# KenHBS/LDA_thesis

Hardware: AMD Instinct MI355X
Metric: million tokens resampled/sec (Gibbs sweep) (higher is better)
Workload: dtype f64-exact (fp32 tier 0 + fp64 tiers: the drawn topic is the fp64 pipeline's)

## Files before the change

### lda_thesis_amd/csrc/kernel_quad.hpp

```cpp
#pragma once

namespace {

constexpr float QM_L = 1.05f * 32.0f * 0x1p-24f, QM_T = 1.05f * 39.0f * 0x1p-24f, QM_P = 1.05f * 37.0f * 0x1p-24f, QM_TOT = 1.05f * 0.25f * 0x1p-24f;
#define QLDS(arr, rho, t) (arr)[(rho) >> 2][t][(rho) & 3]
constexpr int QT = 32;
#ifdef LLDA_QUAD_PRIO
constexpr int QP_TOP = (LLDA_QUAD_PRIO) / 100 % 10, QP_DEC = (LLDA_QUAD_PRIO) / 10 % 10, QP_BULK = (LLDA_QUAD_PRIO) % 10;
#else
constexpr int QP_TOP = 3, QP_DEC = 0, QP_BULK = 2;
#endif
constexpr int QNT = 128;
template <bool B> struct QuadForm { static constexpr bool value = B; };

template <int LB>
struct QuadGeo {
    static constexpr int LPD = 1 << LB;
    static constexpr int G = 2 * LPD;
    static constexpr int KP = 32 * LPD;
    static constexpr int IS = 3 + LB;
    static constexpr int DPW = 64 / LPD;
    static constexpr uint64_t GM = LPD == 64 ? ~0ull : ((1ull << LPD) - 1);
};

template <int LB>
__device__ __forceinline__ int quad_rho(int pos) { return ((pos >> LB) & 0x18) | ((pos & 3) << 1) | ((pos >> 2) & 1); }
constexpr int quad_rho_of(int i, int e, int c) { return 8 * i + 2 * c + e; }

constexpr int QK_LANE = 14;
constexpr uint32_t QK_ZN = (1u << QK_LANE) - 1;
template <int LB> constexpr uint32_t QUAD_KEY_NONE = 0x3Fu << QK_LANE | 31u << 9 | (uint32_t)(QuadGeo<LB>::KP - 1);
static_assert((0x3Fu << QK_LANE | QK_ZN) <= 0x7FFFFFFFu, "the key fits 31 bits");

template <int LB>
__device__ __forceinline__ uint32_t quad_min_key(uint32_t key)
{
    if constexpr (LB == 4)
        asm volatile("s_nop 1\n\tv_min_u32_dpp %0, %0, %0 row_ror:8 row_mask:0xf bank_mask:0xf\n\ts_nop 1\n\t"
                     "v_min_u32_dpp %0, %0, %0 row_ror:4 row_mask:0xf bank_mask:0xf\n\ts_nop 1\n\t"
                     "v_min_u32_dpp %0, %0, %0 row_ror:2 row_mask:0xf bank_mask:0xf\n\ts_nop 1\n\t"
                     "v_min_u32_dpp %0, %0, %0 row_ror:1 row_mask:0xf bank_mask:0xf" : "+v"(key));
    else if constexpr (LB == 3)
        asm volatile("s_nop 1\n\tv_min_u32_dpp %0, %0, %0 row_half_mirror row_mask:0xf bank_mask:0xf\n\ts_nop 1\n\t"
                     "v_min_u32_dpp %0, %0, %0 quad_perm:[1,0,3,2] row_mask:0xf bank_mask:0xf\n\ts_nop 1\n\t"
                     "v_min_u32_dpp %0, %0, %0 quad_perm:[2,3,0,1] row_mask:0xf bank_mask:0xf" : "+v"(key));
    else
        asm volatile("s_nop 1\n\tv_min_u32_dpp %0, %0, %0 quad_perm:[1,0,3,2] row_mask:0xf bank_mask:0xf\n\ts_nop 1\n\t"
                     "v_min_u32_dpp %0, %0, %0 quad_perm:[2,3,0,1] row_mask:0xf bank_mask:0xf" : "+v"(key));
    return key;
}

template <int LB>
struct QuadCounts {
    const int (*s_ndk)[QNT][4];
    const int *s_nk0;
    int t;
    int e;
    int g;
    bool st;
    __device__ __forceinline__ int word(int s) const { return QLDS(s_ndk, 8 * (s >> 2) + 2 * (s & 3) + e, t); }
    __device__ __forceinline__ int nd(int s) const { return word(s) & 0xffff; }
    __device__ __forceinline__ int nk(int s) const
    {
        const int w = word(s);
        return s_nk0[pos_of<QuadGeo<LB>::G, 16>(g, s)] + (w & 0xffff) - (int)((uint32_t)w >> 16);
    }
    __device__ __forceinline__ bool stats() const { return st; }
    __device__ __forceinline__ bool count_unsure() const { return false; }
};

template <int LB, bool PAD>
__device__ __noinline__ int quad_cold(const int (*s_ndk)[QNT][4], const int *s_nk0, int tbase, int w, int f, int zo, uint32_t ra,
                                      uint32_t rb, int lane, int64_t d, const KParams *P)
{
    constexpr int G = QuadGeo<LB>::G;
    const int g = lane & (G - 1);
    int x[16];
    gload_lane_row<G, 16>(P->n_kw, (int64_t)w * QuadGeo<LB>::KP, g, x);
    int lo, so;
    lane_slot_of<G, 16>(zo, lo, so);
#pragma unroll
    for (int s = 0; s < 16; ++s) x[s] -= (g == lo && s == so) ? f : 0;
    const QuadCounts<LB> dc{s_ndk, s_nk0, tbase + (g >> 1), g & 1, g, lane < G};
    if constexpr (PAD) return cold_tiers_acc<G, 16, true, false>(dc, x, P->lab_mask[d * G + g], uniform53(ra, rb), g, lane, P);
    else return cold_tiers_acc<G, 16, false, true>(dc, x, 0xFFFFu, uniform53(ra, rb), g, lane, P);
}

typedef float q_v2f __attribute__((ext_vector_type(2)));
typedef float q_v32f __attribute__((ext_vector_type(32)));

template <int LB, bool PAD = false, bool HOOKS = true>
__device__ __forceinline__ uint64_t quad_draw(const q_v32f &xv, const q_v2f (&pa)[16], float u, float margin_rel, float margin_data, float beta,
                                              int lq, int &zn)
{
    const q_v2f b2 = {beta, beta};
    q_v2f Q[16];
    LLDA_MARK("scores");
#pragma unroll
    for (int a = 0; a < 16; ++a) {
        const q_v2f x2 = {xv[2 * a], xv[2 * a + 1]};
        const q_v2f nb = x2 + b2;
        if (a == 0) Q[0] = nb * pa[0];
        else Q[a] = __builtin_elementwise_fma(nb, pa[a], Q[a - 1]);
    }
    LLDA_MARK("lane_scan");
    __builtin_amdgcn_s_setprio(QP_DEC);
    const float X0 = Q[15].x + Q[15].y;
    float X = X0;
    float tot = X0, prev;
    if constexpr (LB == 4) {
        X += dpp_f32<DPP_ROW_SHR + 1>(X);
        X += dpp_f32<DPP_ROW_SHR + 2>(X);
        X += dpp_f32<DPP_ROW_SHR + 4>(X);
        X += dpp_f32<DPP_ROW_SHR + 8>(X);
        tot += dpp_f32<DPP_ROW_ROR + 8>(tot);
        tot += dpp_f32<DPP_ROW_ROR + 4>(tot);
        tot += dpp_f32<DPP_ROW_ROR + 2>(tot);
        tot += dpp_f32<DPP_ROW_ROR + 1>(tot);
        prev = __int_as_float(__builtin_amdgcn_update_dpp(0, __float_as_int(X), DPP_ROW_SHR + 1, 0xF, 0xF, true));
    } else {
        const float m1 = lq >= 1 ? 1.0f : 0.0f, m2 = lq >= 2 ? 1.0f : 0.0f;
        X = __builtin_fmaf(dpp_f32<DPP_ROW_SHR + 1>(X), m1, X);
        X = __builtin_fmaf(dpp_f32<DPP_ROW_SHR + 2>(X), m2, X);
        if constexpr (LB == 3) {
            const float m4 = lq >= 4 ? 1.0f : 0.0f;
            X = __builtin_fmaf(dpp_f32<DPP_ROW_SHR + 4>(X), m4, X);
            tot += dpp_f32<DPP_HALF_MIRROR>(tot);
        }
        tot += dpp_f32<DPP_XOR1>(tot);
        tot += dpp_f32<DPP_XOR2>(tot);
        prev = dpp_f32<DPP_ROW_SHR + 1>(X) * m1;
    }
    LLDA_MARK("threshold");
    const float t = u * tot;
    const float tg = t - prev;
    const float md = __builtin_fmaf(QM_L, X0, __builtin_fmaf(QM_T, t, __builtin_fmaf(QM_P, prev, QM_TOT * tot)));
    float margin = md;
    if constexpr (HOOKS) margin = __builtin_fmaf(tot, margin_rel, margin_data * md);
    const float lo0 = tg - margin, hi0 = tg + margin;
    LLDA_MARK("search");
    const bool c0 = Q[15].x <= lo0;
    const float dA = c0 ? Q[15].x : 0.0f;
    const float lo = lo0 - dA, hi = hi0 - dA;
    float q[16];
#pragma unroll
    for (int a = 0; a < 16; ++a) q[a] = c0 ? Q[a].y : Q[a].x;
    const bool c5 = q[15] <= lo;
    float ub = c5 ? __int_as_float(0x7f800000) : q[15];
    const bool c1 = q[7] <= lo;
    ub = c1 ? ub : q[7];
    const float m2 = c1 ? q[11] : q[3];
    const float a1 = c1 ? q[9] : q[1], a5 = c1 ? q[13] : q[5];
    const float e0 = c1 ? q[8] : q[0], e2 = c1 ? q[10] : q[2], e4 = c1 ? q[12] : q[4], e6 = c1 ? q[14] : q[6];
    const bool c2 = m2 <= lo;
    ub = c2 ? ub : m2;
    const float m3 = c2 ? a5 : a1;
    const float g0 = c2 ? e4 : e0, g2 = c2 ? e6 : e2;
    const bool c3 = m3 <= lo;
    ub = c3 ? ub : m3;
    const float m4 = c3 ? g2 : g0;
    const bool c4 = m4 <= lo;
    ub = c4 ? ub : m4;
    uint64_t bad_total;
    asm("v_cmp_class_f32_e64 %0, %1, %2" : "=s"(bad_total) : "v"(tot - margin), "v"(0x2FF));
    uint64_t unsure = __ballot(!(ub > hi)) | bad_total;
    LLDA_MARK("pick");
    constexpr uint32_t I1 = 2u << QuadGeo<LB>::IS, I0 = 1u << QuadGeo<LB>::IS;
    const uint32_t p = (c1 ? (I1 | 16u << 9) : 0u) | (c2 ? (I0 | 8u << 9) : 0u) | (c3 ? (2u | 4u << 9) : 0u) |
                       (c4 ? (1u | 2u << 9) : 0u) | (c0 ? (4u | 1u << 9) : 0u) | ((uint32_t)lq << 3) | ((uint32_t)lq << QK_LANE);
    uint32_t key = c5 ? QUAD_KEY_NONE<LB> : p;
    key = quad_min_key<LB>(key);
    zn = (int)(key & QK_ZN);
    if constexpr (PAD) unsure |= __ballot(key == QUAD_KEY_NONE<LB>);
    return unsure;
}

template <int LB, bool PAD = false>
__device__ __forceinline__ uint64_t quad_tier1(const q_v32f &xv, const int (*s_ndk)[QNT][4], const int *s_nk0, int tid, int lq, double u,
                                               double alpha, double beta, double vbeta, double margin_rel, uint32_t vm, int &zn)
{
    double W[QT];
    double run = 0.0;
#pragma unroll
    for (int k = 0; k < QT; ++k) {
        const int e = k >> 4, a = k & 15, i = a >> 2, c = a & 3;
        const int rho = quad_rho_of(i, e, c);
        const int w = QLDS(s_ndk, rho, tid);
        const int nd = w & 0xffff, nk = s_nk0[(i << QuadGeo<LB>::IS) | (lq << 3) | (e << 2) | c] + nd - (int)((uint32_t)w >> 16);
        const double den = (double)nk + vbeta;
        double y = (double)__builtin_amdgcn_rcpf((float)den);
        y = __builtin_fma(__builtin_fma(-den, y, 1.0), y, y);
        y = __builtin_fma(__builtin_fma(-den, y, 1.0), y, y);
        const double ws = ((double)nd + alpha) * (((double)xv[rho] + beta) * y);
        run = run + (((vm >> k) & 1u) ? ws : 0.0);
        W[k] = run;
    }
    constexpr int LPD = QuadGeo<LB>::LPD;
    const double X = group_scan<LPD>(run, lq);
    const double tot = bcast_last<LPD>(X, tid & 63);
    double prev = dpp_f64<DPP_ROW_SHR + 1>(X);
    if constexpr (LB < 4) prev = lq ? prev : 0.0;
    const double tg = u * tot - prev;
    const double margin = tot * margin_rel;
    const double lo = tg - margin, hi = tg + margin;
    int cnt_lo = 0, cnt_hi = 0;
#pragma unroll
    for (int k = 0; k < QT; ++k) {
        cnt_lo += (W[k] <= lo) ? 1 : 0;
        cnt_hi += (W[k] <= hi) ? 1 : 0;
    }
    uint64_t unsure = __ballot((cnt_lo != cnt_hi) || !(tot > 0.0) || !(margin < tot));
    const uint32_t k = (uint32_t)cnt_lo;
    const uint32_t i_ = (k >> 2) & 3u, e_ = (k >> 4) & 1u, c_ = k & 3u;
    const uint32_t p = (i_ << QuadGeo<LB>::IS) | ((uint32_t)lq << 3) | (e_ << 2) | c_ | ((8u * i_ + 2u * c_ + e_) << 9) | ((uint32_t)lq << QK_LANE);
    uint32_t key = cnt_lo >= QT ? QUAD_KEY_NONE<LB> : p;
    key = quad_min_key<LB>(key);
    zn = (int)(key & QK_ZN);
    if constexpr (PAD) unsure |= __ballot(key == QUAD_KEY_NONE<LB>);
    return unsure;
}

struct QuadSite { int v, f, zo, c, zn, lo, so; uint8_t w; };

struct QuadDocLds {
    __attribute__((aligned(16))) int ndk[QT / 4][QNT][4];
    __attribute__((aligned(16))) float pa[QT / 4][QNT][4];
};
static_assert(offsetof(QuadDocLds, pa) == sizeof(int) * QT * QNT && sizeof(int) * QT * QNT < 65536,
              "the factor of a slot is an immediate offset away from its count");

#ifdef QUAD_PROFILE
#define QP_DECL uint32_t qp_t = 0, qp_acc[8] = {0, 0, 0, 0, 0, 0, 0, 0}
#define QP_START() do { __builtin_amdgcn_sched_barrier(0); qp_t = (uint32_t)__builtin_amdgcn_s_memtime(); __builtin_amdgcn_sched_barrier(0); } while (0)
#define QP_MARK(k) do { __builtin_amdgcn_sched_barrier(0); const uint32_t qp_n = (uint32_t)__builtin_amdgcn_s_memtime(); \
                        qp_acc[k] += qp_n - qp_t; qp_t = qp_n; __builtin_amdgcn_sched_barrier(0); } while (0)
#else
#define QP_DECL
#define QP_START()
#define QP_MARK(k)
#endif

template <int LB, bool REC = (LB < 4), bool PAD = false, bool HOOKS = false>
__global__ void __launch_bounds__(QNT, 2) llda_sweep_quad_kernel(const KParams P)
{
    typedef QuadGeo<LB> Geo;
    constexpr int KP = Geo::KP, LPD = Geo::LPD, G = Geo::G, IS = Geo::IS;
    __shared__ int s_nk[KP];
    __shared__ int s_nk0[KP];
    __shared__ QuadDocLds s_doc;
    int (*const s_ndk)[QNT][4] = s_doc.ndk;
    float (*const s_pa)[QNT][4] = s_doc.pa;
    __shared__ float s_u[QNT / LPD][2 * LPD];
    __shared__ __attribute__((aligned(16))) int s_hot[QT][16];
    __shared__ uint16_t s_ent[KP];
    static_assert(LB != 4 || sizeof(s_nk) + sizeof(s_nk0) + sizeof(s_doc) + sizeof(s_u) + sizeof(s_hot) + sizeof(s_ent) <= 40960,
                  "K = 512: the static LDS of a workgroup must leave room for four workgroups on a CU");

    const int tid = threadIdx.x;
    for (int i = tid; i < KP; i += QNT) {
        s_nk[i] = 0;
        s_nk0[i] = P.n_k[i];
        s_ent[i] = (uint16_t)quad_rho<LB>(i);
    }
    for (int i = tid; i < QT * 16; i += QNT) {
        const int so = i >> 4, k = i & 15;
        const int kk = ((so & 1) << 3) | ((so >> 4) << 2) | (((so >> 3) & 1) << 1) | ((so >> 2) & 1);
        s_hot[so][k] = k == kk ? -(1 << (((so >> 1) & 1) << 4)) : 0;
    }
    __syncthreads();

    const int lane = tid & 63, lq = tid & (LPD - 1), row = lane >> LB, grp = tid >> LB;
    const int gbase = lane & (64 - LPD);
    const float vbeta32 = (float)P.vbeta, alpha32 = (float)P.alpha, beta32 = (float)P.beta;

    const int64_t site_base = P.doc_off[0];
    const int32_t *word_b = P.word + site_base, *freq_b = P.freq + site_base, *csc_b = P.csc_pos + site_base;
    int32_t *z_b = P.z + site_base;

    typedef int v4i __attribute__((ext_vector_type(4)));
    QP_DECL;

    auto ndk_of = [&](int sg) -> int * { return &QLDS(s_doc.ndk, sg, tid); };
    auto pa_of = [&](int *nd) -> float * { return (float *)((char *)nd + offsetof(QuadDocLds, pa)); };
    auto update = [&](int sg, int pos, int df) {
        int *const c = ndk_of(sg);
        const int w = *c + df;
        *c = w;
        const int nd = w & 0xffff, nk = s_nk0[pos] + nd - (int)((uint32_t)w >> 16);
        *pa_of(c) = tier0_factor(nd, nk, alpha32, vbeta32);
    };

    for (int it = 0; it < P.dpg; ++it) {
        const int64_t idx = ((int64_t)blockIdx.x * P.dpg + it) * (QNT / LPD) + grp;
        const bool valid = idx < P.D;
        const int64_t ic = valid ? idx : P.D - 1;
        const int64_t d = P.doc_order ? (int64_t)P.doc_order[ic] : ic;
        int64_t s0 = P.doc_off[d];
        int len = valid ? (int)(P.doc_off[d + 1] - s0) : 0;
        if (len <= 0) {
            len = 0;
            s0 = site_base;
        }
        int maxlen, minlen;
        if constexpr (LB == 4) {
            const int l0 = __builtin_amdgcn_readlane(len, 0), l1 = __builtin_amdgcn_readlane(len, 16);
            const int l2 = __builtin_amdgcn_readlane(len, 32), l3 = __builtin_amdgcn_readlane(len, 48);
            maxlen = max(max(l0, l1), max(l2, l3));
            minlen = min(min(l0, l1), min(l2, l3));
        } else {
            int ml = len, nl = len;
#pragma unroll
            for (int m = LPD; m < 64; m <<= 1) {
                ml = max(ml, __shfl_xor(ml, m, 64));
                nl = min(nl, __shfl_xor(nl, m, 64));
            }
            maxlen = __builtin_amdgcn_readfirstlane(ml);
            minlen = __builtin_amdgcn_readfirstlane(nl);
        }
        if (maxlen == 0) continue;

        int32_t *ndk_row = P.n_dk + d * KP;
        const uint32_t vm = PAD ? (uint32_t)P.lab_mask[d * G + 2 * lq] | (uint32_t)P.lab_mask[d * G + 2 * lq + 1] << 16 : ~0u;
        {
            int big = 0, tokens = 0;
#pragma unroll
            for (int i = 0; i < 4; ++i) {
                const v4i a = ((const v4i *)ndk_row)[i * G + 2 * lq], b = ((const v4i *)ndk_row)[i * G + 2 * lq + 1];
                const int r[8] = {a.x, a.y, a.z, a.w, b.x, b.y, b.z, b.w};
#pragma unroll
                for (int j = 0; j < 8; ++j) {
                    const int rho = quad_rho_of(i, j >> 2, j & 3);
                    const int k = s_nk0[(i << IS) + lq * 8 + j];
                    QLDS(s_ndk, rho, tid) = r[j] | (r[j] << 16);
                    QLDS(s_pa, rho, tid) = ((vm >> (16 * (j >> 2) + 4 * i + (j & 3))) & 1u) ? tier0_factor(r[j], k, alpha32, vbeta32) : 0.0f;
                    big |= r[j];
                    tokens += (int)((uint32_t)r[j] & 0xffffu);
                }
            }
#pragma unroll
            for (int m = 1; m < LPD; m <<= 1) tokens += __shfl_xor(tokens, m, LPD);
            if (valid && (((uint32_t)big >> 16) || tokens > 65535) && P.status) atomicOr(P.status, 4);
        }
        const uint32_t gdoc = (uint32_t)(d + P.doc_base);
        const uint32_t sb = (uint32_t)(s0 - site_base) * 4u;
        const int last = len > 0 ? len - 1 : 0;
        auto off_of = [&](int n) { return opaque_u32(sb + (uint32_t)min(n, last) * 4u); };
        auto off_full = [&](int n) { return opaque_u32(sb + (uint32_t)n * 4u); };
        auto load_scalars = [&](QuadSite &R, const uint32_t o) {
            R.v = gload_i32(word_b, o); R.f = gload_i32(freq_b, o); R.c = gload_i32(csc_b, o); R.zo = gload_i32(z_b, o);
        };
        const int32_t *rec_b = REC ? P.site_rec + site_base * 4 : nullptr;
        int pv = 0, pf = 0, pc = 0;
        auto load_rec = [&](int &v, int &f, int &c, const uint32_t o) {
            const v4i r = *(const LLDA_GLOBAL v4i *)((const LLDA_GLOBAL char *)rec_b + (o << 2));
            v = r.x; f = r.y; c = r.z;
        };
        auto decode_old = [&](QuadSite &R) {
            R.lo = (R.zo >> 3) & (LPD - 1);
            R.so = s_ent[R.zo];
            asm("" : "+v"(R.so));
        };
        int xp[16];
        auto load_row16 = [&](const int v, uint8_t &flag) {
#ifdef ABL_NOLOAD
#pragma unroll
            for (int k = 0; k < 16; ++k) xp[k] = ((v + k) & 7) * 0x10001;
            flag = 1;
            return;
#endif
            const LLDA_GLOBAL char *q = (const LLDA_GLOBAL char *)P.n_kw16 + (((uint32_t)v << (IS + 3)) + (uint32_t)lq * 16u);
            const v4i a = *(const LLDA_GLOBAL v4i *)q, b = *(const LLDA_GLOBAL v4i *)(q + 32 * LPD);
            const v4i c = *(const LLDA_GLOBAL v4i *)(q + 16 * LPD), e = *(const LLDA_GLOBAL v4i *)(q + 48 * LPD);
            xp[0] = a.x; xp[1] = a.y; xp[2] = a.z; xp[3] = a.w;
            xp[4] = b.x; xp[5] = b.y; xp[6] = b.z; xp[7] = b.w;
            xp[8] = c.x; xp[9] = c.y; xp[10] = c.z; xp[11] = c.w;
            xp[12] = e.x; xp[13] = e.y; xp[14] = e.z; xp[15] = e.w;
            flag = *(const LLDA_GLOBAL uint8_t *)((const LLDA_GLOBAL char *)P.row16 + (uint32_t)v);
        };
        q_v32f xv;
        auto convert_row = [&](const int v, const uint8_t flag, const int so, const float own) {
            LLDA_MARK("convert");
            const uint64_t wide_w = __ballot(flag == 0);
            if (__builtin_expect(wide_w == 0, 1)) {
#pragma unroll
                for (int k = 0; k < 16; ++k) {
                    const int e = k >> 3, j = (k >> 2) & 1, m = k & 3;
                    const int i = 2 * j + (m >> 1), c = 2 * (m & 1);
                    xv[quad_rho_of(i, e, c)] = (float)((uint32_t)xp[k] & 0xffffu);
                    xv[quad_rho_of(i, e, c + 1)] = (float)((uint32_t)xp[k] >> 16);
                }
            } else {
                LLDA_MARK("rare_wide_row");
                int xi[QT];
#pragma unroll
                for (int t = 0; t < QT; ++t) xi[t] = 0;
                if (flag == 0) {
                    const LLDA_GLOBAL v4i *q = (const LLDA_GLOBAL v4i *)((const LLDA_GLOBAL int32_t *)P.n_kw + ((uint64_t)(uint32_t)v << (IS + 2)));
#pragma unroll
                    for (int i = 0; i < 4; ++i) {
                        const v4i a = q[i * G + 2 * lq], b = q[i * G + 2 * lq + 1];
                        xi[quad_rho_of(i, 0, 0)] = a.x; xi[quad_rho_of(i, 0, 1)] = a.y; xi[quad_rho_of(i, 0, 2)] = a.z; xi[quad_rho_of(i, 0, 3)] = a.w;
                        xi[quad_rho_of(i, 1, 0)] = b.x; xi[quad_rho_of(i, 1, 1)] = b.y; xi[quad_rho_of(i, 1, 2)] = b.z; xi[quad_rho_of(i, 1, 3)] = b.w;
                    }
                }
#pragma unroll
                for (int k = 0; k < 16; ++k) {
                    const int e = k >> 3, j = (k >> 2) & 1, m = k & 3;
                    const int i = 2 * j + (m >> 1), c = 2 * (m & 1);
                    const int ra_ = quad_rho_of(i, e, c), rb_ = quad_rho_of(i, e, c + 1);
                    xv[ra_] = flag == 0 ? (float)xi[ra_] : (float)((uint32_t)xp[k] & 0xffffu);
                    xv[rb_] = flag == 0 ? (float)xi[rb_] : (float)((uint32_t)xp[k] >> 16);
                }
#pragma unroll
                for (int r = 0; r < QT; ++r) xv[r] -= (flag == 0 && so == r) ? own : 0.0f;
            }
        };
        auto remove_own_packed = [&](const int so, const int own) {
            LLDA_MARK("own_removal");
            __builtin_assume((uint32_t)own < 65536u);
            const v4i *hot = (const v4i *)&s_hot[so][0];
#pragma unroll
            for (int j = 0; j < 4; ++j) {
                const v4i h = hot[j];
                xp[4 * j] += __mul24(h.x, own); xp[4 * j + 1] += __mul24(h.y, own);
                xp[4 * j + 2] += __mul24(h.z, own); xp[4 * j + 3] += __mul24(h.w, own);
            }
        };

        QuadSite R0, R1, R2;
        int wq = 0;
        if constexpr (REC) {
            load_rec(R0.v, R0.f, R0.c, off_of(0)); R0.zo = gload_i32(z_b, off_of(0));
            load_rec(R1.v, R1.f, R1.c, off_of(1)); R1.zo = gload_i32(z_b, off_of(1));
            load_rec(pv, pf, pc, off_of(2));
        } else {
            load_scalars(R0, off_of(0));
            load_scalars(R1, off_of(1));
            wq = gload_i32(word_b, off_of(2));
        }
        R0.zn = R1.zn = R2.zn = R2.f = R2.c = R2.lo = R2.so = R2.w = 0;
        R2.v = REC ? pv : wq;
        R2.zo = gload_i32(z_b, off_of(2));
        load_row16(R0.v, R0.w);
        uint32_t r0 = 0, r1 = 0, r2 = 0, r3 = 0;
        decode_old(R0);
        decode_old(R1);
        if (len > 0 && lq == R0.lo) update(R0.so, R0.zo, -R0.f);
        remove_own_packed(R0.so, (len > 0 && lq == R0.lo) ? R0.f : 0);
        convert_row(R0.v, R0.w, R0.so, (len > 0 && lq == R0.lo) ? (float)R0.f : 0.0f);
        load_row16(R1.v, R1.w);

        auto site = [&](auto form, const int n, QuadSite &cur, QuadSite &nxt, QuadSite &prv) {
            constexpr bool FULL = decltype(form)::value;
            const bool act = FULL || n < len, more = FULL || n + 1 < len;
            auto off = [&](int m) { if constexpr (FULL) return off_full(m); else return off_of(m); };
            const int f = cur.f, zo = cur.zo;
            QP_START();
            if constexpr (FULL) { LLDA_MARK("site_top"); } else { LLDA_MARK("site_top_masked"); }
            LLDA_MARK("lds_factors");
            __builtin_amdgcn_s_setprio(QP_TOP);
            q_v2f pa[16];
#pragma unroll
            for (int a = 0; a < 16; ++a) {
                pa[a].x = QLDS(s_pa, 2 * a, tid);
                pa[a].y = QLDS(s_pa, 2 * a + 1, tid);
            }
            LLDA_MARK("rng");
            if ((n & (2 * LPD - 1)) == 0) {
                LLDA_MARK("rare_philox");
                r0 = (uint32_t)(n >> 1) + (uint32_t)lq; r1 = gdoc; r2 = P.stream_id; r3 = P.sweep;
                philox4x32_10(r0, r1, r2, r3, P.key0, P.key1);
                s_u[grp][2 * lq] = (float)(r0 >> 5) * 0x1p-27f;
                s_u[grp][2 * lq + 1] = (float)(r2 >> 5) * 0x1p-27f;
                LLDA_MARK("rng");
            }
            const float u32 = s_u[grp][n & (2 * LPD - 1)];
            QP_MARK(0);
            int zn;
            uint64_t unsure;
            if constexpr (HOOKS) unsure = quad_draw<LB, PAD, true>(xv, pa, u32, P.margin0_rel, P.margin0_data, beta32, lq, zn);
            else unsure = quad_draw<LB, PAD, false>(xv, pa, u32, 0.0f, 1.0f, beta32, lq, zn);
            if constexpr (!FULL) unsure &= __ballot(act);
            QP_MARK(1);
            LLDA_MARK("cold_check");
            if (__builtin_expect(unsure != 0, 0)) {
                LLDA_MARK("rare_cold");
                const int holder = (n >> 1) & (LPD - 1);
                const uint32_t ra_l = (n & 1) ? r2 : r0, rb_l = (n & 1) ? r3 : r1;
                const int bp_h = (gbase | holder) << 2;
                const uint32_t ra = (uint32_t)__builtin_amdgcn_ds_bpermute(bp_h, (int)ra_l), rb = (uint32_t)__builtin_amdgcn_ds_bpermute(bp_h, (int)rb_l);
                const uint64_t t0_w = unsure;
                if (lq == 0 && ((t0_w >> gbase) & Geo::GM) && P.status) atomicAdd(P.status + 1, 1);
                int z1;
                uint64_t still = ((!HOOKS || P.margin_rel < 1.0 ? quad_tier1<LB, PAD>(xv, s_ndk, s_nk0, tid, lq, uniform53(ra, rb), P.alpha, P.beta, P.vbeta,
                                                                                  P.margin_rel, vm, z1) : ~0ull) | __ballot(cur.w == 0));
                if constexpr (!FULL) still &= __ballot(act);
                const bool mine0 = ((t0_w >> gbase) & Geo::GM) != 0;
                zn = mine0 ? z1 : zn;
                uint32_t rows = 0;
#pragma unroll
                for (int r = 0; r < Geo::DPW; ++r)
                    rows |= (((t0_w >> (LPD * r)) & Geo::GM) && ((still >> (LPD * r)) & Geo::GM)) ? (1u << r) : 0u;
                rows = (uint32_t)__builtin_amdgcn_readfirstlane((int)rows);
                while (__builtin_expect(rows != 0, 0)) {
                    const int r = __builtin_ctz(rows);
                    rows &= rows - 1;
                    const int src = r * LPD;
                    const int zo_r = __builtin_amdgcn_readlane(zo, src);
                    int zc = quad_cold<LB, PAD>(s_ndk, s_nk0, (tid & 64) + src, __builtin_amdgcn_readlane(cur.v, src),
                                       __builtin_amdgcn_readlane(f, src), zo_r, (uint32_t)__builtin_amdgcn_readlane((int)ra, src),
                                       (uint32_t)__builtin_amdgcn_readlane((int)rb, src), lane,
                                       (int64_t)__builtin_amdgcn_readlane((int)d, src),
                                       (const KParams *)__builtin_amdgcn_kernarg_segment_ptr());
                    if (__builtin_expect(zc < 0, 0)) {
                        zc = zo_r;
                        if (lane == 0 && P.status) atomicOr(P.status, 1);
                    }
                    zn = (row == r) ? (zc | quad_rho<LB>(zc) << 9) : zn;
                }
            }
            QP_MARK(2);
            LLDA_MARK("decode");

            {
                const int zpos = zn & 511, sn = zn >> 9, ln = (zn >> 3) & (LPD - 1);
                cur.zn = zpos;
                uint32_t cword = (uint32_t)zo | ((uint32_t)zpos << 16);
                asm volatile("" : "+v"(cword));
                const bool own_new = act && lq == ln, own_old = more && lq == nxt.lo;
                const uint64_t both_w = __builtin_amdgcn_ballot_w64(own_new) & __builtin_amdgcn_ballot_w64(own_old);
                const int sg = own_new ? sn : own_old ? nxt.so : 0;
                const int ps = own_new ? zpos : own_old ? nxt.zo : (lq << 3);
                const int df = own_new ? f : own_old ? -nxt.f : 0;
                LLDA_MARK("count_update");
                int *const cg = ndk_of(sg);
                const int w0 = *cg, k0 = s_nk0[ps];
                QP_MARK(3);
                LLDA_MARK("scalars");
                __builtin_amdgcn_s_setprio(QP_BULK);
                int w_next;
                if constexpr (REC) {
                    prv.v = w_next = pv; prv.f = pf; prv.c = pc;
                    cur.zo = gload_i32(z_b, off(n + 3));
                    load_rec(pv, pf, pc, off(n + 3));
                } else {
                    w_next = prv.v;
                    prv.f = gload_i32(freq_b, off(n + 2)); prv.c = gload_i32(csc_b, off(n + 2));
                    cur.v = gload_i32(word_b, off(n + 3)); cur.zo = gload_i32(z_b, off(n + 3));
                }
                decode_old(prv);
                QP_MARK(4);
                remove_own_packed(nxt.so, (more && lq == nxt.lo) ? nxt.f : 0);
                convert_row(nxt.v, nxt.w, nxt.so, (more && lq == nxt.lo) ? (float)nxt.f : 0.0f);
                QP_MARK(5);
                LLDA_MARK("row_prefetch");
                load_row16(w_next, prv.w);
                LLDA_MARK("count_update");
                const int w = w0 + df;
                *cg = w;
                const int nd = w & 0xffff, nk = k0 + nd - (int)((uint32_t)w >> 16);
                *pa_of(cg) = tier0_factor(nd, nk, alpha32, vbeta32);
                if (__builtin_expect(both_w != 0, 0)) {
                    LLDA_MARK("rare_second_update");
                    if (own_new && own_old) update(nxt.so, nxt.zo, -nxt.f);
                }
#ifndef ABL_NOCOMMIT
                {
                    LLDA_MARK("commit");
                    const uint32_t zoff = opaque_u32(sb + (uint32_t)n * 4u);
                    const uint32_t loff = (uint32_t)cur.c << 2;
                    if (lq == 0 && act) {
                        gstore_i32(z_b, zoff, zpos);
                        gstore_i32((int32_t *)P.commit_log, loff, (int)cword);
                    }
                }
#endif
            }
            LLDA_MARK("loop");
            QP_MARK(6);
        };
        int n = 0;
        for (; n + 5 < minlen; n += 3) {
            site(QuadForm<true>{}, n, R0, R1, R2);
            site(QuadForm<true>{}, n + 1, R1, R2, R0);
            site(QuadForm<true>{}, n + 2, R2, R0, R1);
        }
        for (;; n += 3) {
            site(QuadForm<false>{}, n, R0, R1, R2);
            if (n + 1 >= maxlen) break;
            site(QuadForm<false>{}, n + 1, R1, R2, R0);
            if (n + 2 >= maxlen) break;
            site(QuadForm<false>{}, n + 2, R2, R0, R1);
            if (n + 3 >= maxlen) break;
        }

#ifdef QUAD_PROFILE
        if (blockIdx.x == 0 && tid == 0 && P.status) {
#pragma unroll
            for (int k = 0; k < 8; ++k) atomicAdd(P.status + 8 + k, (int)qp_acc[k]);
            atomicAdd(P.status + 16, maxlen);
        }
#endif
        if (valid && len > 0) {
#pragma unroll
            for (int i = 0; i < 4; ++i) {
                int o[8];
#pragma unroll
                for (int j = 0; j < 8; ++j) {
                    const int w = QLDS(s_ndk, quad_rho_of(i, j >> 2, j & 3), tid);
                    o[j] = w & 0xffff;
                    const int dl = o[j] - (int)((uint32_t)w >> 16);
                    if (dl) atomicAdd(&s_nk[(i << IS) + lq * 8 + j], dl);
                }
                v4i a = {o[0], o[1], o[2], o[3]}, b = {o[4], o[5], o[6], o[7]};
                ((v4i *)ndk_row)[i * G + 2 * lq] = a;
                ((v4i *)ndk_row)[i * G + 2 * lq + 1] = b;
            }
        }
    }

    __syncthreads();
    for (int i = tid; i < KP; i += QNT) {
        const int dl = s_nk[i];
        if (dl) atomicAdd(P.n_k_delta + i, dl);
    }
}

template <int G>
__global__ void __launch_bounds__(256) llda_pack_rows16_all_kernel(const int32_t *__restrict__ n_kw, uint16_t *__restrict__ out,
                                                                   uint8_t *__restrict__ row16, int64_t V)
{
    const int64_t t = (int64_t)blockIdx.x * 256 + threadIdx.x;
    const int64_t w = t / (2 * G);
    if (w >= V) return;
    const int c = (int)(t & (2 * G - 1)), j = c / G, g = c & (G - 1);
    const int4 *src = reinterpret_cast<const int4 *>(n_kw + w * (int64_t)(G * 16));
    const int4 a = src[(2 * j) * G + g], b = src[(2 * j + 1) * G + g];
    const int m = a.x | a.y | a.z | a.w | b.x | b.y | b.z | b.w;
    const uint64_t bal = __ballot((unsigned)m > 0xffffu);
    const int first = (int)(threadIdx.x & 63) & ~(2 * G - 1);
    const bool wide = G == 32 ? bal != 0 : ((bal >> first) & ((1ull << (2 * G % 64)) - 1)) != 0;
    uint4 o;
    o.x = ((uint32_t)a.x & 0xffffu) | ((uint32_t)a.y << 16);
    o.y = ((uint32_t)a.z & 0xffffu) | ((uint32_t)a.w << 16);
    o.z = ((uint32_t)b.x & 0xffffu) | ((uint32_t)b.y << 16);
    o.w = ((uint32_t)b.z & 0xffffu) | ((uint32_t)b.w << 16);
    reinterpret_cast<uint4 *>(out + w * (int64_t)(G * 16))[(2 * j + (g & 1)) * (G / 2) + (g >> 1)] = o;
    if (c == 0) row16[w] = wide ? 0 : 1;
}

}
```

Baseline: 9288.

## Prefetch next document's offsets and overlap n_dk row load with site prologue

Computes the next document's index and doc_off bounds one iteration ahead so they are ready when the loop advances. Moves the global load of the document's n_dk row after the first site-scalar loads, so it overlaps with load_row16 before the LDS fill runs. Changes the document-to-block mapping from contiguous per-block chunks to a grid-strided interleave, and adds profiling counters for the per-document prologue and epilogue. The cost is extra registers for the prefetched values and sched_barriers that constrain the compiler's scheduling.

```diff
diff --git a/lda_thesis_amd/csrc/kernel_quad.hpp b/lda_thesis_amd/csrc/kernel_quad.hpp
--- a/lda_thesis_amd/csrc/kernel_quad.hpp
+++ b/lda_thesis_amd/csrc/kernel_quad.hpp
@@ -230,7 +230,7 @@
               "the factor of a slot is an immediate offset away from its count");
 
 #ifdef QUAD_PROFILE
-#define QP_DECL uint32_t qp_t = 0, qp_acc[8] = {0, 0, 0, 0, 0, 0, 0, 0}
+#define QP_DECL uint32_t qp_t = 0, qp_acc[10] = {0, 0, 0, 0, 0, 0, 0, 0, 0, 0}; int qp_sites = 0, qp_groups = 0
 #define QP_START() do { __builtin_amdgcn_sched_barrier(0); qp_t = (uint32_t)__builtin_amdgcn_s_memtime(); __builtin_amdgcn_sched_barrier(0); } while (0)
 #define QP_MARK(k) do { __builtin_amdgcn_sched_barrier(0); const uint32_t qp_n = (uint32_t)__builtin_amdgcn_s_memtime(); \
                         qp_acc[k] += qp_n - qp_t; qp_t = qp_n; __builtin_amdgcn_sched_barrier(0); } while (0)
@@ -257,28 +257,51 @@
                   "K = 512: the static LDS of a workgroup must leave room for four workgroups on a CU");
 
     const int tid = threadIdx.x;
-    for (int i = tid; i < KP; i += QNT) {
-        s_nk[i] = 0;
-        s_nk0[i] = P.n_k[i];
-        s_ent[i] = (uint16_t)quad_rho<LB>(i);
+    QP_DECL;
+    QP_START();
+    const int lane = tid & 63, lq = tid & (LPD - 1), row = lane >> LB, grp = tid >> LB;
+    auto doc_of = [&](int it, bool &valid) -> uint32_t {
+        const int64_t idx = ((int64_t)it * gridDim.x + blockIdx.x) * (QNT / LPD) + grp;
+        valid = it < P.dpg && idx < P.D;
+        const int64_t ic = valid ? idx : P.D - 1;
+        return P.doc_order ? (uint32_t)P.doc_order[ic] : (uint32_t)ic;
+    };
+    bool valid_n;
+    uint32_t d_n = doc_of(0, valid_n);
+    {
+        int nk0[KP / QNT];
+#pragma unroll
+        for (int j = 0; j < KP / QNT; ++j) nk0[j] = P.n_k[tid + j * QNT];
+#pragma unroll
+        for (int j = 0; j < KP / QNT; ++j) {
+            const int i = tid + j * QNT;
+            s_nk[i] = 0;
+            s_nk0[i] = nk0[j];
+            s_ent[i] = (uint16_t)quad_rho<LB>(i);
+        }
     }
     for (int i = tid; i < QT * 16; i += QNT) {
         const int so = i >> 4, k = i & 15;
         const int kk = ((so & 1) << 3) | ((so >> 4) << 2) | (((so >> 3) & 1) << 1) | ((so >> 2) & 1);
         s_hot[so][k] = k == kk ? -(1 << (((so >> 1) & 1) << 4)) : 0;
     }
+    const int64_t site_base = P.doc_off[0];
+    uint32_t sb_n;
+    int len_n;
+    {
+        const int64_t o0 = P.doc_off[(int64_t)d_n], o1 = P.doc_off[(int64_t)d_n + 1];
+        sb_n = (uint32_t)(o0 - site_base);
+        len_n = (int)(o1 - o0);
+    }
     __syncthreads();
 
-    const int lane = tid & 63, lq = tid & (LPD - 1), row = lane >> LB, grp = tid >> LB;
     const int gbase = lane & (64 - LPD);
     const float vbeta32 = (float)P.vbeta, alpha32 = (float)P.alpha, beta32 = (float)P.beta;
 
-    const int64_t site_base = P.doc_off[0];
     const int32_t *word_b = P.word + site_base, *freq_b = P.freq + site_base, *csc_b = P.csc_pos + site_base;
     int32_t *z_b = P.z + site_base;
 
     typedef int v4i __attribute__((ext_vector_type(4)));
-    QP_DECL;
 
     auto ndk_of = [&](int sg) -> int * { return &QLDS(s_doc.ndk, sg, tid); };
     auto pa_of = [&](int *nd) -> float * { return (float *)((char *)nd + offsetof(QuadDocLds, pa)); };
@@ -291,15 +314,13 @@
     };
 
     for (int it = 0; it < P.dpg; ++it) {
-        const int64_t idx = ((int64_t)blockIdx.x * P.dpg + it) * (QNT / LPD) + grp;
-        const bool valid = idx < P.D;
-        const int64_t ic = valid ? idx : P.D - 1;
-        const int64_t d = P.doc_order ? (int64_t)P.doc_order[ic] : ic;
-        int64_t s0 = P.doc_off[d];
-        int len = valid ? (int)(P.doc_off[d + 1] - s0) : 0;
+        const bool valid = valid_n;
+        const int64_t d = d_n;
+        uint32_t sb = sb_n * 4u;
+        int len = valid ? len_n : 0;
         if (len <= 0) {
             len = 0;
-            s0 = site_base;
+            sb = 0;
         }
         int maxlen, minlen;
         if constexpr (LB == 4) {
@@ -317,32 +338,16 @@
             maxlen = __builtin_amdgcn_readfirstlane(ml);
             minlen = __builtin_amdgcn_readfirstlane(nl);
         }
-        if (maxlen == 0) continue;
+        d_n = doc_of(it + 1, valid_n);
+        if (maxlen == 0) {
+            const int64_t o0 = P.doc_off[(int64_t)d_n], o1 = P.doc_off[(int64_t)d_n + 1];
+            sb_n = (uint32_t)(o0 - site_base);
+            len_n = (int)(o1 - o0);
+            continue;
+        }
 
         int32_t *ndk_row = P.n_dk + d * KP;
-        const uint32_t vm = PAD ? (uint32_t)P.lab_mask[d * G + 2 * lq] | (uint32_t)P.lab_mask[d * G + 2 * lq + 1] << 16 : ~0u;
-        {
-            int big = 0, tokens = 0;
-#pragma unroll
-            for (int i = 0; i < 4; ++i) {
-                const v4i a = ((const v4i *)ndk_row)[i * G + 2 * lq], b = ((const v4i *)ndk_row)[i * G + 2 * lq + 1];
-                const int r[8] = {a.x, a.y, a.z, a.w, b.x, b.y, b.z, b.w};
-#pragma unroll
-                for (int j = 0; j < 8; ++j) {
-                    const int rho = quad_rho_of(i, j >> 2, j & 3);
-                    const int k = s_nk0[(i << IS) + lq * 8 + j];
-                    QLDS(s_ndk, rho, tid) = r[j] | (r[j] << 16);
-                    QLDS(s_pa, rho, tid) = ((vm >> (16 * (j >> 2) + 4 * i + (j & 3))) & 1u) ? tier0_factor(r[j], k, alpha32, vbeta32) : 0.0f;
-                    big |= r[j];
-                    tokens += (int)((uint32_t)r[j] & 0xffffu);
-                }
-            }
-#pragma unroll
-            for (int m = 1; m < LPD; m <<= 1) tokens += __shfl_xor(tokens, m, LPD);
-            if (valid && (((uint32_t)big >> 16) || tokens > 65535) && P.status) atomicOr(P.status, 4);
-        }
         const uint32_t gdoc = (uint32_t)(d + P.doc_base);
-        const uint32_t sb = (uint32_t)(s0 - site_base) * 4u;
         const int last = len > 0 ? len - 1 : 0;
         auto off_of = [&](int n) { return opaque_u32(sb + (uint32_t)min(n, last) * 4u); };
         auto off_full = [&](int n) { return opaque_u32(sb + (uint32_t)n * 4u); };
@@ -441,13 +446,48 @@
         R0.zn = R1.zn = R2.zn = R2.f = R2.c = R2.lo = R2.so = R2.w = 0;
         R2.v = REC ? pv : wq;
         R2.zo = gload_i32(z_b, off_of(2));
+        __builtin_amdgcn_sched_barrier(0);
+        v4i nd[8];
+#pragma unroll
+        for (int i = 0; i < 4; ++i) {
+            nd[2 * i] = ((const v4i *)ndk_row)[i * G + 2 * lq];
+            nd[2 * i + 1] = ((const v4i *)ndk_row)[i * G + 2 * lq + 1];
+        }
+        const uint32_t vm = PAD ? (uint32_t)P.lab_mask[d * G + 2 * lq] | (uint32_t)P.lab_mask[d * G + 2 * lq + 1] << 16 : ~0u;
+        __builtin_amdgcn_sched_barrier(0);
+        int64_t o0 = P.doc_off[(int64_t)d_n], o1 = P.doc_off[(int64_t)d_n + 1];
         load_row16(R0.v, R0.w);
+        __builtin_amdgcn_sched_barrier(0);
+        {
+            int big = 0, tokens = 0;
+#pragma unroll
+            for (int i = 0; i < 4; ++i) {
+                const v4i a = nd[2 * i], b = nd[2 * i + 1];
+                const int r[8] = {a.x, a.y, a.z, a.w, b.x, b.y, b.z, b.w};
+#pragma unroll
+                for (int j = 0; j < 8; ++j) {
+                    const int rho = quad_rho_of(i, j >> 2, j & 3);
+                    const int k = s_nk0[(i << IS) + lq * 8 + j];
+                    QLDS(s_ndk, rho, tid) = r[j] | (r[j] << 16);
+                    QLDS(s_pa, rho, tid) = ((vm >> (16 * (j >> 2) + 4 * i + (j & 3))) & 1u) ? tier0_factor(r[j], k, alpha32, vbeta32) : 0.0f;
+                    big |= r[j];
+                    tokens += (int)((uint32_t)r[j] & 0xffffu);
+                }
+            }
+#pragma unroll
+            for (int m = 1; m < LPD; m <<= 1) tokens += __shfl_xor(tokens, m, LPD);
+            if (valid && (((uint32_t)big >> 16) || tokens > 65535) && P.status) atomicOr(P.status, 4);
+        }
         uint32_t r0 = 0, r1 = 0, r2 = 0, r3 = 0;
         decode_old(R0);
         decode_old(R1);
         if (len > 0 && lq == R0.lo) update(R0.so, R0.zo, -R0.f);
         remove_own_packed(R0.so, (len > 0 && lq == R0.lo) ? R0.f : 0);
         convert_row(R0.v, R0.w, R0.so, (len > 0 && lq == R0.lo) ? (float)R0.f : 0.0f);
+        asm volatile("" : "+v"(o0), "+v"(o1));
+        sb_n = (uint32_t)(o0 - site_base);
+        len_n = (int)(o1 - o0);
+        asm volatile("" : "+v"(sb_n), "+v"(len_n));
         load_row16(R1.v, R1.w);
 
         auto site = [&](auto form, const int n, QuadSite &cur, QuadSite &nxt, QuadSite &prv) {
@@ -580,6 +620,7 @@
             QP_MARK(6);
         };
         int n = 0;
+        QP_MARK(8);
         for (; n + 5 < minlen; n += 3) {
             site(QuadForm<true>{}, n, R0, R1, R2);
             site(QuadForm<true>{}, n + 1, R1, R2, R0);
@@ -595,11 +636,9 @@
         }
 
 #ifdef QUAD_PROFILE
-        if (blockIdx.x == 0 && tid == 0 && P.status) {
-#pragma unroll
-            for (int k = 0; k < 8; ++k) atomicAdd(P.status + 8 + k, (int)qp_acc[k]);
-            atomicAdd(P.status + 16, maxlen);
-        }
+        qp_sites += maxlen;
+        ++qp_groups;
+        QP_START();
 #endif
         if (valid && len > 0) {
 #pragma unroll
@@ -617,7 +656,18 @@
                 ((v4i *)ndk_row)[i * G + 2 * lq + 1] = b;
             }
         }
-    }
+        QP_MARK(9);
+    }
+#ifdef QUAD_PROFILE
+    if (blockIdx.x == 0 && tid == 0 && P.status) {
+#pragma unroll
+        for (int k = 0; k < 8; ++k) atomicAdd(P.status + 8 + k, (int)qp_acc[k]);
+        atomicAdd(P.status + 16, qp_sites);
+        atomicAdd(P.status + 17, (int)qp_acc[8]);
+        atomicAdd(P.status + 18, (int)qp_acc[9]);
+        atomicAdd(P.status + 19, qp_groups);
+    }
+#endif
 
     __syncthreads();
     for (int i = tid; i < KP; i += QNT) {
```

Result: no change. 9285 (-0.0%).
